# Daniel-Liu-c0deb0t/block-aligner

Hardware: AMD Instinct MI355X
Metric: GCUPS (DP cells/s) on 10 kbp DNA X-drop batch; bit-exact score+CIGAR vs AVX2 (higher is better)
Workload: dtype i16 (saturating lane scores) + i32 block offsets

## Files before the change

block_aligner_amd/csrc/ba_host.cpp:

```cpp
#include <hip/hip_runtime.h>

#include <algorithm>
#include <functional>
#include <cmath>
#include <cstdarg>
#include <cstdio>
#include <cstdlib>
#include <cstring>
#include <map>
#include <memory>
#include <string>
#include <vector>
#include <atomic>
#include <chrono>
#include <thread>

#include "../../include/block_aligner_hip.h"
#include "aa_matrices.inc"
#include "ba_extend.h"
#include "ba_stats.h"
#include "ba_params.h"

using ba::BatchParams;
using ba::BlockRec;
// ... 1500 lines not shown
        } else (void)hipGetLastError();
        out = (uint32_t*)at.devicePointer;
    }
    if (!out) {
        if (!b->compact.p) {
            b->compact_cap = std::max<uint64_t>(b->cap_cig / 3, 1u << 20);
            if (b->compact.alloc(b->compact_cap * 4)) return 1;
        }
        out = b->compact.as<uint32_t>(); cap = b->compact_cap;
    }
    HIP_TRY(ba_launch_cigar_offsets_and_compact(b->stream, b->cig_ops.as<uint32_t>(), b->cig_off.as<uint64_t>(), b->cig_len.as<uint32_t>(),
                                                b->h_order.empty() ? nullptr : b->dev_of.as<uint32_t>(), b->compact_off.as<uint64_t>(), out,
                                                b->h_total, cap, b->n));
    b->compacted = true; b->compact_host = pinned_out; b->compact_used_cap = cap;
    return 0;
}
int ba_batch_cigars(BaBatch* b, uint32_t* runs, uint64_t capacity) {
    if (!b) return fail("null batch");
    if (!(b->mode & BA_TRACE)) return fail("batch was created without BA_TRACE");
    if (!b->ran) return fail("ba_batch_run has not been called");
    HIP_TRY(hipSetDevice(b->device));
    if (b->compacted && b->retried == 0) {
        const unsigned long long total = *(volatile unsigned long long*)b->h_total;
        if (total <= b->compact_used_cap) {
            if (total > capacity) return fail("cigar buffer too small: need %llu entries", total);
            if (b->compact_host) { if (runs != b->compact_host && total) memcpy(runs, b->compact_host, total * 4); }
            else if (total) HIP_TRY(hipMemcpy(runs, b->compact.p, total * 4, hipMemcpyDeviceToHost));
            return 0;
        }
    }
    std::vector<uint32_t> len(b->n);
    if (d2h(b->cig_len, len.data(), b->n)) return 1;
    std::vector<uint64_t> out_off(b->n);
    uint64_t total = 0;
    if (b->h_order.empty()) for (uint32_t p = 0; p < b->n; p++) { out_off[p] = total; total += len[p]; }
    else {
        std::vector<uint32_t> dev_of(b->n);
        for (uint32_t s = 0; s < b->n; s++) dev_of[b->h_order[s]] = s;
        for (uint32_t p = 0; p < b->n; p++) { out_off[dev_of[p]] = total; total += len[dev_of[p]]; }
    }
    if (total > capacity) return fail("cigar buffer too small: need %llu entries", (unsigned long long)total);
    if (total == 0) return 0;
    DevBuf d_off, d_out;
    if (d_off.alloc(b->n * 8) || d_out.alloc(total * 4)) return 1;
    HIP_TRY(hipMemcpy(d_off.p, out_off.data(), b->n * 8, hipMemcpyHostToDevice));
    HIP_TRY(ba_launch_compact_cigars(b->stream, b->cig_ops.as<uint32_t>(), b->cig_off.as<uint64_t>(), b->cig_len.as<uint32_t>(),
                                     d_off.as<uint64_t>(), d_out.as<uint32_t>(), b->n));
    HIP_TRY(hipStreamSynchronize(b->stream));
    HIP_TRY(hipMemcpy(runs, d_out.p, total * 4, hipMemcpyDeviceToHost));
    return 0;
}
#ifdef BA_DEV
int ba_dev_lane_scan(int form, const int16_t* x, uint32_t n_cells, int gap_extend, int16_t* out) {
    if (form < 0 || form > 4 || !x || !out) return fail("ba_dev_lane_scan: bad arguments");
    const uint32_t per_wave = form <= 1 ? 512u : (form == 2 ? 128u : (form == 3 ? 64u : 32u));
    if (n_cells == 0 || n_cells % per_wave) return fail("ba_dev_lane_scan: %u cells are not whole waves of %u", n_cells, per_wave);
    if (gap_extend > 0 || gap_extend < -128) return fail("ba_dev_lane_scan: gap_extend %d", gap_extend);
    DevBuf dx, dout;
    if (dx.alloc((size_t)n_cells * 2) || dout.alloc((size_t)n_cells * 2)) return 1;
    HIP_TRY(hipMemcpy(dx.p, x, (size_t)n_cells * 2, hipMemcpyHostToDevice));
    HIP_TRY(ba_launch_lane_kat(nullptr, form, dx.as<short>(), dout.as<short>(), gap_extend, n_cells / per_wave));
    HIP_TRY(hipDeviceSynchronize());
    HIP_TRY(hipMemcpy(out, dout.p, (size_t)n_cells * 2, hipMemcpyDeviceToHost));
    return 0;
}
#endif
int ba_batch_prof(BaBatch* b, uint64_t out[128]) {
    if (!b) return fail("null batch");
    HIP_TRY(hipMemcpy(out, b->prof.p, 1024, hipMemcpyDeviceToHost));
    return 0;
}
int ba_batch_info(BaBatch* b, uint64_t out[4]) {
    if (!b) return fail("null batch");
    out[0] = (uint64_t)b->grid * b->wpw; out[1] = b->lds / b->wpw; out[2] = b->trace.bytes; out[3] = b->pool_bytes;
    return 0;
}
int ba_batch_spec_cells(BaBatch* b, uint64_t* cells) {
    if (!b || !cells) return fail("null argument");
    if (!b->ran) return fail("ba_batch_run has not been called");
    HIP_TRY(hipSetDevice(b->device));
    HIP_TRY(hipMemcpy(cells, (const char*)b->prof.p + 60 * 8, 8, hipMemcpyDeviceToHost));
    return 0;
}
int ba_batch_kernel(BaBatch* b) { return !b ? -1 : (b->small ? 3 : (b->quad ? 2 : (b->multi ? 1 : 0))); }
int ba_batch_geometry(BaBatch* b) { return !b ? -1 : (int)b->geom; }
int ba_batch_retried(BaBatch* b) { return b ? (int)b->retried : -1; }
int ba_batch_stats(BaBatch* b, BaAlignStats* out) {
    if (!b) return fail("null batch");
    if (!out) return fail("null argument");
    if (batch_stats_device(b, true)) return 1;
    HIP_TRY(hipMemcpy(out, b->stats.p, (size_t)b->n * sizeof(ba::AlignStats), hipMemcpyDeviceToHost));
    return 0;
}
int ba_batch_stats_ms(BaBatch* b, float* ms) {
    if (!b || !ms) return fail("null argument");
    *ms = b->stats_ms;
    return 0;
}
void ba_batch_destroy(BaBatch* b) { delete b; }

BaExtendBatch* ba_extend_batch_create(int kind, const void* matrix, Gaps gaps, SizeRange size, int32_t x_drop, uint32_t mode, const uint8_t* pool,
                                      const uint64_t* q_off, const uint32_t* q_len, const uint64_t* r_off, const uint32_t* r_len,
                                      const uint32_t* q_seed, const uint32_t* r_seed, const uint32_t* seed_len, const uint8_t* strand, uintptr_t n_seeds) {
    ExtSet S;
    if (!matrix) { fail("null argument"); return nullptr; }
    if (ext_check_params(kind, gaps, size, x_drop, mode) || ext_plan(kind, pool, q_off, q_len, r_off, r_len, q_seed, r_seed, seed_len, strand, n_seeds, S)) return nullptr;
    if (ensure_device()) return nullptr;
    std::unique_ptr<BaExtendBatch> e(new BaExtendBatch);
// ... 833 lines not shown
```

block_aligner_amd/csrc/ba_kernels.hip:

```cpp
#include "ba_driver.hpp"

#ifndef BA_KIND
#error "define BA_KIND"
#endif
#ifndef BA_PMAX
#error "define BA_PMAX"
#endif

#ifndef BA_SPECIAL
#define BA_SPECIAL 0
#endif

#define BA_CAT_(a, b, c, d) a##b##c##d
#define BA_CAT(a, b, c, d) BA_CAT_(a, b, c, d)
#if BA_BIG && BA_SPECIAL
#define BA_LAUNCH BA_CAT(ba_launch_bigs_k, BA_KIND, _p, BA_PMAX)
#define BA_OCC BA_CAT(ba_occupancy_bigs_k, BA_KIND, _p, BA_PMAX)
#elif BA_BIG
#define BA_LAUNCH BA_CAT(ba_launch_big_k, BA_KIND, _p, BA_PMAX)
#define BA_OCC BA_CAT(ba_occupancy_big_k, BA_KIND, _p, BA_PMAX)
#elif BA_SPECIAL
#define BA_LAUNCH BA_CAT(ba_launch_s_k, BA_KIND, _p, BA_PMAX)
#define BA_OCC BA_CAT(ba_occupancy_s_k, BA_KIND, _p, BA_PMAX)
#else
// ... 258 lines not shown
}
#endif

#if BA_PMAX == 1 && !BA_SPECIAL && !BA_BIG
#include "ba_quad.hpp"
template <bool TRACE, bool XDROP>
static hipError_t quad_grid(unsigned* grid) {
    const unsigned lds = ba::lds_table_bytes_h(BA_KIND) + ba::WAVES_PER_WG * 4 * ba::QUAD_SLOT_BYTES;
    int per_cu = 0, dev = 0;
    hipError_t e = hipOccupancyMaxActiveBlocksPerMultiprocessor(&per_cu, ba::k_quad<BA_KIND, TRACE, XDROP>, ba::WAVES_PER_WG * 64, lds);
    if (e != hipSuccess) return e;
    hipDeviceProp_t prop;
    if ((e = hipGetDevice(&dev)) != hipSuccess || (e = hipGetDeviceProperties(&prop, dev)) != hipSuccess) return e;
    if (per_cu < 1) per_cu = 1;
    if (per_cu * ba::WAVES_PER_WG > 32) per_cu = 32 / ba::WAVES_PER_WG;
    *grid = (unsigned)(prop.multiProcessorCount * per_cu);
    return hipSuccess;
}
template <bool TRACE, bool XDROP>
static hipError_t launch_quad(unsigned grid, hipStream_t s, const ba::BatchParams& bp) {
    const unsigned lds = ba::lds_table_bytes_h(BA_KIND) + ba::WAVES_PER_WG * 4 * ba::QUAD_SLOT_BYTES;
    ba::k_quad<BA_KIND, TRACE, XDROP><<<dim3(grid), dim3(ba::WAVES_PER_WG * 64), lds, s>>>(bp);
    return hipGetLastError();
}
extern "C" hipError_t BA_CAT(ba_launch_quad_k, BA_KIND, , )(int trace, int xdrop, unsigned grid, hipStream_t s, const ba::BatchParams* bp) {
    if (trace) return xdrop ? launch_quad<true, true>(grid, s, *bp) : launch_quad<true, false>(grid, s, *bp);
    return xdrop ? launch_quad<false, true>(grid, s, *bp) : launch_quad<false, false>(grid, s, *bp);
}
extern "C" hipError_t BA_CAT(ba_quad_grid_k, BA_KIND, , )(int trace, int xdrop, unsigned* grid) {
    if (trace) return xdrop ? quad_grid<true, true>(grid) : quad_grid<true, false>(grid);
    return xdrop ? quad_grid<false, true>(grid) : quad_grid<false, false>(grid);
}
#endif

#if BA_KIND == 0 && BA_PMAX == 1 && !BA_SPECIAL && !BA_BIG
__global__ void __launch_bounds__(64) k_traceback(const ba::BatchParams bp) {
    using namespace ba;
    __shared__ uint32_t words[4096];
    uint32_t st = 0, n = 0;
    if (bp.flags & (F_LOCAL | F_FQS)) {
        if (lane_id() == 0)
            n = traceback(bp.blocks + (uint64_t)bp.tb_slot * bp.blocks_stride, bp.tb_nblocks, bp.trace_arena + (uint64_t)bp.tb_slot * bp.trace_stride, bp.tb_i,
                          bp.tb_j, bp.pool + bp.q_off[0], bp.pool + bp.r_off[0], bp.flags, bp.cig_ops, bp.cig_off[0], bp.cig_off[1], &st);
    } else
        n = walk_wave<false>(bp.blocks + (uint64_t)bp.tb_slot * bp.blocks_stride, bp.tb_nblocks, bp.trace_arena + (uint64_t)bp.tb_slot * bp.trace_stride, bp.tb_i,
                             bp.tb_j, bp.pool + bp.q_off[0], bp.pool + bp.r_off[0], (bp.flags & F_CIGAR_EQ) != 0, bp.cig_ops, bp.cig_off[0], bp.cig_off[1], &st,
                             words, 4096u);
    if (lane_id() == 0) { bp.cig_len[0] = n; bp.status[0] = st; }
}

__global__ void __launch_bounds__(64) k_lane_kat(int form, const short* __restrict__ x, short* __restrict__ out, int gap_extend) {
    using namespace ba;
    const int lane = lane_id();
    if (form <= 1) {
        const short* xi = x + (size_t)blockIdx.x * 512 + lane * 8;
        int xr[4], r[4];
#pragma unroll
        for (int k = 0; k < 4; k++) xr[k] = pk((int)xi[2 * k], (int)xi[2 * k + 1]);
        const int ge2 = splat(gap_extend);
#pragma unroll
        for (int k = 0; k < 4; k++) r[k] = scan8_inreg(xr[k], ge2);
        int G[4], cs;
        if (form == 0) {
            const MultiConsts mc = make_multi_consts(lane & 15, gap_extend);
#pragma unroll
            for (int k = 0; k < 4; k++) G[k] = mc.G[k];
            scan8_chain(r, G[0]);
            cs = multi_carry(r[3], mc);
        } else {
            const SmallConsts mc = make_small_consts(lane & 3, gap_extend);
#pragma unroll
            for (int k = 0; k < 4; k++) G[k] = mc.G[k];
            scan8_chain(r, G[0]);
            cs = small_carry(r[3], mc, lane & 3);
        }
        short* oi = out + (size_t)blockIdx.x * 512 + lane * 8;
#pragma unroll
        for (int k = 0; k < 4; k++) { const int v = scan8_apply(r[k], cs, G[k], k == 3); oi[2 * k] = as_s(v).x; oi[2 * k + 1] = as_s(v).y; }
    } else {
        const int nl = form == 2 ? 64 : (form == 3 ? 32 : 16);
        const size_t base = (size_t)blockIdx.x * (size_t)(2 * nl);
        const int xv = lane < nl ? pk((int)x[base + 2 * lane], (int)x[base + 2 * lane + 1]) : 0;
        const FillConsts fc = make_fill_consts(lane, 0, gap_extend);
        const int v = form == 2 ? fast_scan<64>(xv, fc) : (form == 3 ? fast_scan<32>(xv, fc) : fast_scan<16>(xv, fc));
        if (lane < nl) { out[base + 2 * lane] = as_s(v).x; out[base + 2 * lane + 1] = as_s(v).y; }
    }
}
extern "C" hipError_t ba_launch_lane_kat(hipStream_t s, int form, const short* x, short* out, int gap_extend, unsigned waves) {
    k_lane_kat<<<dim3(waves), dim3(64), 0, s>>>(form, x, out, gap_extend);
    return hipGetLastError();
}

constexpr int WALK_WAVES = 4;
__global__ void __launch_bounds__(WALK_WAVES * 64) k_walk(const ba::BatchParams bp) {
    extern __shared__ __attribute__((aligned(16))) unsigned char walk_lds[];
    ba::traceback_all(bp, (uint32_t)ba::F_CIGAR_EQ, walk_lds + ((uint32_t)threadIdx.x >> 6) * ba::TB_LDS_BYTES);
}

__global__ void __launch_bounds__(WALK_WAVES * 64) k_walk_l2(const ba::BatchParams bp) {
    extern __shared__ __attribute__((aligned(16))) unsigned char walk_lds[];
    ba::traceback_all<true>(bp, (uint32_t)ba::F_CIGAR_EQ, walk_lds + ((uint32_t)threadIdx.x >> 6) * ba::TB_LDS_BYTES_L2);
}

__global__ void __launch_bounds__(WALK_WAVES * 64) k_walk_loc(const ba::BatchParams bp) {
    extern __shared__ __attribute__((aligned(16))) unsigned char walk_lds[];
    ba::traceback_all<true, true>(bp, (uint32_t)ba::F_CIGAR_EQ, walk_lds + ((uint32_t)threadIdx.x >> 6) * ba::TB_LDS_BYTES_LOC);
}
// ... 126 lines not shown
```

block_aligner_amd/csrc/ba_multi.hpp:

```cpp
#pragma once
#include "ba_quad.hpp"

namespace ba {
#ifndef MQ_SOLO_PRIO
#define MQ_SOLO_PRIO 2
#endif

template <int N>
__device__ __forceinline__ int row_bcast(int v) { return __builtin_amdgcn_update_dpp(v, v, 0x150 + N, 0xf, 0xf, false); }
__device__ __forceinline__ int row_shl1_keep(int last, int src) { return __builtin_amdgcn_update_dpp(last, src, 0x101, 0xf, 0xf, false); }
__device__ __forceinline__ int splat_hi(int x) { const s16x2 t = as_s(x); return as_i(s16x2{t.y, t.y}); }
__device__ __forceinline__ int splat_lo(int x) { const s16x2 t = as_s(x); return as_i(s16x2{t.x, t.x}); }

__device__ __forceinline__ int sel_mask(unsigned long long m, int a, int b) {
    int r;
    asm("v_cndmask_b32_e64 %0, %1, %2, %3" : "=v"(r) : "v"(b), "v"(a), "s"(m));
    return r;
}

template <int SL> __device__ __forceinline__ int slot_first(int v) {
    if constexpr (SL == 16) return row_bcast<0>(v);
    else if constexpr (SL == 64) return __builtin_amdgcn_readfirstlane(v);
    else return __builtin_amdgcn_ds_bpermute((lane_id() & 32) << 2, v);
}
template <int SL> __device__ __forceinline__ int slot_last(int v) {
    if constexpr (SL == 16) return row_bcast<15>(v);
    else if constexpr (SL == 64) return __builtin_amdgcn_readlane(v, 63);
    else return __builtin_amdgcn_ds_bpermute(((lane_id() & 32) + 31) << 2, v);
}
template <int SL> __device__ __forceinline__ int slot_shr1_z(int v, int l) {
    if constexpr (SL == 16) return row_shr1_z(v);
    else if constexpr (SL == 64) return wave_shr1_z(v);
    else { const int t = wave_shr1_z(v); return l == 0 ? 0 : t; }
}
template <int SL> __device__ __forceinline__ int slot_shl1_keep(int last, int src, int l) {
    if constexpr (SL == 16) return row_shl1_keep(last, src);
    else { const int t = __builtin_amdgcn_update_dpp(last, src, 0x130, 0xf, 0xf, false); return l == SL - 1 ? last : t; }
}

struct MultiConsts {
    int G[4];
    int laneKG, lanem1KG;
    int w0;
};

__device__ __forceinline__ MultiConsts make_multi_consts(int l, int gx) {
    MultiConsts mc;
    mc.laneKG = l * 8 * gx; mc.lanem1KG = l ? (l - 1) * 8 * gx : -32768;
#pragma unroll
    for (int k = 0; k < 4; k++) mc.G[k] = pk(max(-32768, (2 * k + 1) * gx), max(-32768, (2 * k + 2) * gx));
    mc.w0 = pk(0, l == 0 ? 0 : ((l & 1) ? max(-32768, 8 * l * gx) : 4 * gx));
    return mc;
}
template <int SL = 16>
__device__ __forceinline__ int multi_carry(int r3, const MultiConsts& mc, int l = 0) {
    if constexpr (SL == 16) {
        const int pm = wave_prefix_max16((int)as_s(r3).y - mc.laneKG);
        return vmax(scan8_splat_lo(add_row_shr1(pm, mc.lanem1KG)), mc.w0);
    } else {
        const int pm = SL == 64 ? wave_prefix_max((int)as_s(r3).y - mc.laneKG) : wave_prefix_max32((int)as_s(r3).y - mc.laneKG);
        const int cin = add_shr1(pm, mc.lanem1KG);
        return vmax(scan8_splat_lo(l == 0 ? -32768 : cin), mc.w0);
    }
}

struct MultiOut { int mx, act_max8, pas_max8, corner_new; };

template <int KIND, bool TRACE, int SPM = 0, int SL = 16>
__device__ __forceinline__ void multi_rect(const char* table, const FillConsts& fc, const MultiConsts& mc, int l, int (&Ad)[4], int (&Ac)[4],
                                           int (&Pd)[4], int (&Pr)[4], uint2 vb, uint32_t cb_lo, uint32_t cb_hi, int corner, int off_add,
                                           uint32_t* __restrict__ tout, bool store, MultiOut& o, int rz2 = 0, bool fqs_row0 = false, int* zout = nullptr) {
    uint32_t zacc[2] = {0, 0};
    const int offa = splat(off_add);
    int d[4], c[4], pd[4], pr[4];
#pragma unroll
    for (int k = 0; k < 4; k++) {
        d[k] = adds(Ad[k], offa); c[k] = adds(Ac[k], offa); pd[k] = adds(Pd[k], offa); pr[k] = adds(Pr[k], offa);
    }
    o.corner_new = slot_first<SL>(pd[3]) >> 16;
    ScoreKey<KIND> key[4];
#pragma unroll
    for (int k = 0; k < 4; k++) {
        const uint32_t w = k < 2 ? vb.x : vb.y;
        key[k] = make_key<KIND>((int)((w >> (16 * (k & 1))) & 0xffu), (int)((w >> (16 * (k & 1) + 8)) & 0xffu));
    }
    uint32_t kb[4] = {0, 0, 0, 0}, cbs_lo = 0, cbs_hi = 0;
    if constexpr (KIND == KIND_NUC) {
        const uint32_t tb = (uint32_t)(uintptr_t)table, k01 = nuc_keys2(vb.x), k23 = nuc_keys2(vb.y);
        kb[0] = add_word(k01, tb, 0); kb[1] = add_word(k01, tb, 1); kb[2] = add_word(k23, tb, 0); kb[3] = add_word(k23, tb, 1);
        cbs_lo = nuc_col_offsets(cb_lo); cbs_hi = nuc_col_offsets(cb_hi);
    }
    int dmax[4] = {0, 0, 0, 0}, tacc[8] = {0, 0, 0, 0, 0, 0, 0, 0};
    int nvD[4] = {0, 0, 0, 0}, nvR[4] = {0, 0, 0, 0};
    int holdD = 0, holdR = 0;
#pragma unroll
    for (int j = 0; j < STEP; j++) {
        const int cb = (int)(((j < 4 ? cb_lo : cb_hi) >> (8 * (j & 3))) & 0xffu);
        int sc[4];
#pragma unroll
        for (int k = 0; k < 4; k++) {
            if constexpr (KIND == KIND_NUC) sc[k] = lds_read_i32(add_byte(j < 4 ? cbs_lo : cbs_hi, kb[k], j));
            else sc[k] = fetch_score<KIND>(table, key[k], cb);
        }
        int prev = slot_shr1_z<SL>(d[3], l);
        if (j == 0) prev = l == 0 ? (int)((uint32_t)corner << 16) : prev;
        int d00[4];
        d00[0] = __builtin_amdgcn_alignbit(d[0], prev, 16);
#pragma unroll
        for (int k = 1; k < 4; k++) d00[k] = __builtin_amdgcn_alignbit(d[k], d[k - 1], 16);
        int d11[4], copen[4], cn[4], x[4], r[4];
#pragma unroll
        for (int k = 0; k < 4; k++) {
            d11[k] = adds(d00[k], sc[k]);
            if (SPM == 2 && k == 0) d11[0] = fqs_row0 ? (int)(((uint32_t)d11[0] & 0xffff0000u) | ((uint32_t)rz2 & 0xffffu)) : d11[0];
            if (SPM == 1) d11[k] = vmax(d11[k], rz2);
            copen[k] = adds(d[k], fc.go2);
            cn[k] = vmax(adds(c[k], fc.ge2), copen[k]);
            d11[k] = vmax(d11[k], cn[k]);
            x[k] = adds(d11[k], fc.ome2);
            r[k] = scan8_inreg(x[k], fc.ge2);
        }
        scan8_chain(r, mc.G[0]);
        const int cs = multi_carry<SL>(r[3], mc, l);
        int dn[4];
        uint32_t sC[4], sR[4], sCo[4], sRo[4];
#pragma unroll
        for (int k = 0; k < 4; k++) {
            r[k] = scan8_apply(r[k], cs, mc.G[k], k == 3);
            dn[k] = vmax(d11[k], r[k]);
            if (TRACE) {
                sC[k] = (uint32_t)subs(cn[k], dn[k]); sR[k] = (uint32_t)subs(r[k], dn[k]); sCo[k] = (uint32_t)subs(copen[k], cn[k]); sRo[k] = (uint32_t)subs(x[k], r[k]);
            }
            dmax[k] = vmax(dmax[k], dn[k]);
            d[k] = dn[k]; c[k] = cn[k];
        }
        if (TRACE && SPM == 1) {
#pragma unroll
            for (int p2 = 0; p2 < 2; p2++) {
                const uint32_t pZ = (uint32_t)__builtin_amdgcn_perm(subs(rz2, dn[2 * p2 + 1]), subs(rz2, dn[2 * p2]), 0x0b0a0908);
                zacc[p2] |= pZ & (0x01010101u << j);
            }
        }
        if (TRACE) {
#pragma unroll
            for (int p2 = 0; p2 < 2; p2++) {
                const uint32_t pC = (uint32_t)__builtin_amdgcn_perm((int)sC[2 * p2 + 1], (int)sC[2 * p2], 0x0b0a0908), pR = (uint32_t)__builtin_amdgcn_perm((int)sR[2 * p2 + 1], (int)sR[2 * p2], 0x0b0a0908);
                const uint32_t pCo = (uint32_t)__builtin_amdgcn_perm((int)sCo[2 * p2 + 1], (int)sCo[2 * p2], 0x0b0a0908), pRo = (uint32_t)__builtin_amdgcn_perm((int)sRo[2 * p2 + 1], (int)sRo[2 * p2], 0x0b0a0908);
                const uint32_t lo2 = bfi(0x55555555u, pC, pR), hi2 = bfi(0x55555555u, pCo, pRo);
                const uint32_t nib = bfi(0x33333333u, lo2, hi2);
                if (j & 1) tacc[2 * (j >> 1) + p2] = (int)bfi(0xF0F0F0F0u, nib, (uint32_t)tacc[2 * (j >> 1) + p2]);
                else tacc[2 * (j >> 1) + p2] = (int)nib;
            }
        }
        if (j & 1) { nvD[j >> 1] = __builtin_amdgcn_perm(dn[3], holdD, 0x07060302); nvR[j >> 1] = __builtin_amdgcn_perm(r[3], holdR, 0x07060302); }
        else { holdD = dn[3]; holdR = r[3]; }
    }
    if (TRACE) {
#ifndef MQ_X_NOTRSTORE
        if (store) { *(int4*)tout = int4{tacc[0], tacc[1], tacc[2], tacc[3]}; *(int4*)(tout + 4) = int4{tacc[4], tacc[5], tacc[6], tacc[7]}; }
#else
        asm volatile("" :: "v"(tacc[0]), "v"(tacc[1]), "v"(tacc[2]), "v"(tacc[3]), "v"(tacc[4]), "v"(tacc[5]), "v"(tacc[6]), "v"(tacc[7]));
#endif
    }
#pragma unroll
    for (int k = 0; k < 4; k++) {
        Pd[k] = slot_shl1_keep<SL>(nvD[k], pd[k], l); Pr[k] = slot_shl1_keep<SL>(nvR[k], pr[k], l);
        Ad[k] = d[k]; Ac[k] = c[k];
    }
    {
        const int ma = vmax(vmax(d[0], d[1]), vmax(d[2], d[3])), mb = vmax(vmax(Pd[0], Pd[1]), vmax(Pd[2], Pd[3]));
        const s16x2 sa = as_s(ma), sb = as_s(mb);
        const int xa = vmax(ma, as_i(s16x2{sa.y, sa.x})), xb = vmax(mb, as_i(s16x2{sb.y, sb.x}));
        const s16x2 rr = as_s(slot_first<SL>(__builtin_amdgcn_perm(xb, xa, 0x05040100)));
        o.act_max8 = rr.x; o.pas_max8 = rr.y;
    }
    const int mm = vmax(vmax(dmax[0], dmax[1]), vmax(dmax[2], dmax[3]));
    const int m32 = max(mm & 0xffff, (int)((uint32_t)mm >> 16));
    o.mx = slot_last<SL>(SL == 16 ? wave_prefix_max16(m32) : (SL == 64 ? wave_prefix_max(m32) : wave_prefix_max32(m32)));
    if constexpr (TRACE && SPM == 1) { zout[0] = (int)~zacc[0]; zout[1] = (int)~zacc[1]; }
}

enum { MR_PAIR = 0, MR_BEST_I, MR_BEST_J, MR_CELLS_LO, MR_CELLS_HI, MR_BUDGET, MR_STATUS, MR_TSLOT, MR_SI, MR_SJ, MR_DIR, MR_PREV_DIR, MR_OFF, MR_OFF_MAX,
       MR_BEST_MAX, MR_Y_DROP, MR_X_ITER, MR_D_CORNER, MR_NSTEPS, MR_TRACE_TOP, MR_NBLOCKS, MR_SEL, MR_WORDS };
__device__ __forceinline__ int mq_load(const char* p) { return __hip_atomic_load((const int*)p, BA_RLX_AGENT); }

#ifndef MQ_PARTIAL_MB
#define MQ_PARTIAL_MB 256
#endif
#ifndef MQ_WAVES_EU
#define MQ_WAVES_EU 4
#endif
template <int PMAX, int KIND, bool TRACE, bool XDROP, int SPM = 0, int MBP = 128, int WPW = WAVES_PER_WG, int EU = MQ_WAVES_EU>
__global__ void __launch_bounds__(WPW * 64, (PMAX >= 16 ? 2 : EU)) k_multi(const BatchParams bp) {
    constexpr uint32_t MB = (uint32_t)MBP;
    constexpr int SL = MBP / 8, NSLOT = 64 / SL;
    constexpr uint32_t ALLM = (1u << NSLOT) - 1u;
    constexpr uint32_t ARR = 2u * MB, BUFL = 4u * ARR, BUFA = BUFL + 64u, SLOTA = 2u * BUFA + 128u;
    static_assert((MBP == 128 || MBP == 256 || MBP == 512) && NSLOT * SLOTA <= MQ_WAVE_BYTES && NSLOT * 2u * BUFL <= MQ_LDS_SCALARS && (MBP == 128 || SPM == 0), "k_multi slot geometry");
    static_assert(MBP != 128 || (BUFA == MQ_BUF_BYTES && SLOTA == MQ_SLOT_BYTES), "ba_params.h");
    constexpr uint32_t MQ_TW = (STEP * MB / 8) * (SPM == 1 ? 2u : 1u);
    constexpr int TB_LB = SPM ? (int)TB_LANE_BYTES_LOC : (int)TB_LANE_BYTES_L2;
    constexpr uint32_t TB_MASK = SPM ? ~0u : (uint32_t)F_CIGAR_EQ;
    extern __shared__ __attribute__((aligned(16))) char smem[];
    const int lane = lane_id(), l = lane & (SL - 1), g = lane / SL;
    const int wave = uni((int)threadIdx.x >> 6);
    {
        char* tab = smem;
        if (KIND == KIND_NUC) {
            nuc_table_fill(tab, bp.matrix, (int)threadIdx.x, WPW * 64);
        } else {
            const int nbytes = KIND == KIND_AA ? 27 * 32 : 2;
            for (int k = (int)threadIdx.x; k < nbytes; k += WPW * 64) tab[k] = (char)bp.matrix[k];
        }
    }
    __syncthreads();
    constexpr uint32_t LCLS = (uint32_t)PMAX * 128u;
    constexpr uint32_t ab = lds_array_bytes_h(LCLS);
    char* base = smem + lds_table_bytes_h(KIND) + (uint32_t)wave * mq_wave_bytes_h(LCLS);
    WaveLds L;
    L.D_col = (short*)(base + 0 * ab); L.C_col = (short*)(base + 1 * ab);
    L.D_row = (short*)(base + 2 * ab); L.R_row = (short*)(base + 3 * ab);
    L.misc = (short*)(base + 4 * ab);
    L.table = smem;
    const int gx = bp.gap_extend;
    const uint32_t stride = bp.tb_stride;
    const bool batch_traceback = TRACE && stride > 0;
#if defined(BA_TIMING) || defined(BA_ENDHIST)
    if (bp.prof && blockIdx.x == 0 && wave == 1 && is_lane(0)) atomicMax(bp.prof + 43, (unsigned long long)__builtin_amdgcn_s_memrealtime());
#endif
#ifdef BA_TIMING
    unsigned long long t_solo = 0, t_quad = 0, t_wait = 0, n_solo = 0, n_quad = 0;
#endif
// ... 159 lines not shown
                        uint32_t f = 0, head = 0;
                        if ((uint32_t)lane < bp.slots_per_wave) f = __hip_atomic_load(bp.slot_free + s_slot + lane, BA_RLX_AGENT);
                        if (is_lane(0)) head = __hip_atomic_load(bp.tb_ctrl + 32, BA_RLX_AGENT);
                        const unsigned long long fm = __ballot(f != 0);
                        if (fm) {
                            s_slot += (uint32_t)__builtin_ctzll(fm);
                            if (is_lane(0)) __hip_atomic_store(bp.slot_free + s_slot, 0u, BA_RLX_AGENT);
                            break;
                        }
                        head = (uint32_t)uni((int)head);
                        if (head != seen) { seen = head; idle_n = 0; }
                        else if ((++idle_n & 2047u) == 0 && traceback_help_one<TB_LB>(bp, TB_MASK, (unsigned char*)base)) idle_n = 0;
                        __builtin_amdgcn_s_sleep(64);
                    }
#ifdef BA_TIMING
                    t_wait += __builtin_amdgcn_s_memtime() - tw_a;
#endif
                } else if (TRACE) {
                    s_slot += (uint32_t)solo;
                }
            } else {
                const int rv = lane < MR_WORDS ? mq_load(rec + 4 * lane) : 0;
#define BA_W(v, k) __builtin_amdgcn_readlane(v, k)
                const uint32_t s_sel = (uint32_t)BA_W(rv, MR_SEL);
                const char* live_b = smem_s + (s_sel ^ 1u) * BUFA; const char* ck_b = smem_s + s_sel * BUFA;
                const int cv = lane < 16 ? mq_load(ck_b + BUFL + 4 * lane) : 0;
                s_pair = (uint32_t)BA_W(rv, MR_PAIR); s_slot = (uint32_t)BA_W(rv, MR_TSLOT);
                st.si = (uint32_t)BA_W(rv, MR_SI); st.sj = (uint32_t)BA_W(rv, MR_SJ); st.dir = BA_W(rv, MR_DIR); st.prev_dir = BA_W(rv, MR_PREV_DIR);
                st.off = BA_W(rv, MR_OFF); st.off_max = BA_W(rv, MR_OFF_MAX); st.best_max = BA_W(rv, MR_BEST_MAX);
                st.y_drop_iter = (uint32_t)BA_W(rv, MR_Y_DROP); st.x_drop_iter = BA_W(rv, MR_X_ITER); st.D_corner = BA_W(rv, MR_D_CORNER);
                st.trace_top = (uint32_t)BA_W(rv, MR_TRACE_TOP); st.nblocks = (uint32_t)BA_W(rv, MR_NBLOCKS);
                const uint32_t ns = (uint32_t)BA_W(rv, MR_NSTEPS);
                st.best_i = (uint32_t)BA_W(rv, MR_BEST_I); st.best_j = (uint32_t)BA_W(rv, MR_BEST_J);
                st.cells = ((unsigned long long)(uint32_t)BA_W(rv, MR_CELLS_LO) | ((unsigned long long)(uint32_t)BA_W(rv, MR_CELLS_HI) << 32)) + (unsigned long long)ns * (STEP * MB);
                const uint32_t bud = (uint32_t)BA_W(rv, MR_BUDGET);
                st.step_budget = bud > ns ? bud - ns : 1u;
                st.status = (uint32_t)BA_W(rv, MR_STATUS);
                const int flag = BA_W(cv, 0);
                const bool ck_pre = flag != 0;
                st.ck_i = (uint32_t)BA_W(cv, 1); st.ck_j = (uint32_t)BA_W(cv, 2); st.ck_off = BA_W(cv, 3);
                st.ck_tt = (uint32_t)BA_W(cv, 4) + (flag ? MQ_TW : 0u); st.ck_nb = (uint32_t)BA_W(cv, 5) + (flag ? 1u : 0u);
                const int ck_dir = BA_W(cv, 6), ck_offadd = BA_W(cv, 7), ck_corner = BA_W(cv, 8);
#undef BA_W
                {
                    int reg[16], ckr[16];
                    const bool lr = st.dir == DIR_RIGHT, cr = ck_dir == DIR_RIGHT;
                    const uint32_t oAd = (lr ? 0u : 2 * ARR) + l * 16, oAc = (lr ? ARR : 3 * ARR) + l * 16, oPd = (lr ? 2 * ARR : 0u) + l * 16, oPr = (lr ? 3 * ARR : ARR) + l * 16;
                    const uint32_t cAd = (cr ? 0u : 2 * ARR) + l * 16, cAc = (cr ? ARR : 3 * ARR) + l * 16, cPd = (cr ? 2 * ARR : 0u) + l * 16, cPr = (cr ? 3 * ARR : ARR) + l * 16;
#pragma unroll
                    for (int k = 0; k < 4; k++) {
                        reg[k] = mq_load(live_b + oAd + 4 * k); reg[4 + k] = mq_load(live_b + oAc + 4 * k); reg[8 + k] = mq_load(live_b + oPd + 4 * k); reg[12 + k] = mq_load(live_b + oPr + 4 * k);
                        ckr[k] = mq_load(ck_b + cAd + 4 * k); ckr[4 + k] = mq_load(ck_b + cAc + 4 * k); ckr[8 + k] = mq_load(ck_b + cPd + 4 * k); ckr[12 + k] = mq_load(ck_b + cPr + 4 * k);
                    }
                    al.import_slot(reg, ckr, s_pair, ck_pre || MB < max_size, ck_pre, ck_dir, ck_offadd, ck_corner, st.ck_i, st.ck_j, st.best_i, st.best_j, st.ck_off);
                }
            }
            al.trace = bp.trace_arena + (uint64_t)s_slot * bp.trace_stride;
            al.blocks = bp.blocks + (uint64_t)s_slot * bp.blocks_stride;
            int keepv = 0;
            park<0>(keepv, (int)live_m); park<1>(keepv, (int)pend_m); park<2>(keepv, (int)w_next); park<3>(keepv, (int)w_end);
            park<4>(keepv, (more ? 1 : 0) | (fresh ? 2 : 0) | (to_end ? 4 : 0) | (drain ? 8 : 0)); park<5>(keepv, solo); park<6>(keepv, (int)s_pair); park<7>(keepv, (int)s_slot);
            BA_TSTAMP(tr_a);
            __builtin_amdgcn_s_setprio(MQ_SOLO_PRIO);
            st = al.run(s_pair, s_slot, batch_traceback, nullptr, fresh ? MM_FRESH : MM_RESUME, st, !to_end, !fresh && !to_end);
            __builtin_amdgcn_s_setprio(0);
            live_m = (uint32_t)unpark<0>(keepv); pend_m = (uint32_t)unpark<1>(keepv); w_next = (uint32_t)unpark<2>(keepv); w_end = (uint32_t)unpark<3>(keepv);
            { const int fl = unpark<4>(keepv); more = fl & 1; fresh = fl & 2; to_end = fl & 4; drain = fl & 8; }
            solo = unpark<5>(keepv); s_pair = (uint32_t)unpark<6>(keepv); s_slot = (uint32_t)unpark<7>(keepv);
            char* const smem_s2 = (char*)coldp_big() + (uint64_t)fill_wave_of() * MQ_WAVE_BYTES + (uint32_t)solo * SLOTA;
            char* const rec2 = smem_s2 + 2 * BUFA;
#ifdef BA_TIMING
            {
                const unsigned long long tr_b = __builtin_amdgcn_s_memtime();
                al.prof[45] += tr_b - tr_a; al.prof[46] += fresh ? 1 : 0;
                if (bp.prof && is_lane(0)) {
                    for (int k = 0; k < 48; k++) if (k != 17 && !(k >= 20 && k < 32) && !(k >= 40 && k < 44)) atomicAdd(bp.prof + k, al.prof[k]);
                    atomicAdd(bp.prof + (fresh ? 56 : (to_end ? 58 : 57)), tr_b - tr_a);
                }
            }
#endif
            pend_m &= ~(1u << solo);
            if (st.exited) {
                const bool rgt = st.dir == DIR_RIGHT;
                if (lane < SL) {
                    const int l8 = 8 * l;
                    const int4 a_d = *(const int4*)((rgt ? L.D_col : L.D_row) + l8), a_c = *(const int4*)((rgt ? L.C_col : L.R_row) + l8);
                    const int4 p_d = *(const int4*)((rgt ? L.D_row : L.D_col) + l8), p_r = *(const int4*)((rgt ? L.R_row : L.C_col) + l8);
                    char* b1 = smem_s2 + BUFA;
                    *(int4*)(b1 + l * 16) = a_d; *(int4*)(b1 + ARR + l * 16) = a_c; *(int4*)(b1 + 2 * ARR + l * 16) = p_d; *(int4*)(b1 + 3 * ARR + l * 16) = p_r;
                    if (MB < max_size) {
                        char* b0 = smem_s2;
                        *(int4*)(b0 + l * 16) = *(const int4*)(L.D_col + MB + l8); *(int4*)(b0 + ARR + l * 16) = *(const int4*)(L.C_col + MB + l8);
                        *(int4*)(b0 + 2 * ARR + l * 16) = *(const int4*)(L.D_row + MB + l8); *(int4*)(b0 + 3 * ARR + l * 16) = *(const int4*)(L.R_row + MB + l8);
                    }
                }
                if (is_lane(0)) {
                    char* b0 = smem_s2;
                    *(int4*)(b0 + BUFL) = int4{0, (int)st.ck_i, (int)st.ck_j, st.ck_off}; *(int4*)(b0 + BUFL + 16) = int4{(int)st.ck_tt, (int)st.ck_nb, DIR_RIGHT, 0};
                    *(int*)(b0 + BUFL + 32) = 0;
                    int* rc = (int*)rec2;
                    rc[MR_PAIR] = (int)s_pair; rc[MR_BEST_I] = (int)st.best_i; rc[MR_BEST_J] = (int)st.best_j; rc[MR_CELLS_LO] = (int)(uint32_t)st.cells; rc[MR_CELLS_HI] = (int)(uint32_t)(st.cells >> 32);
                    rc[MR_BUDGET] = (int)st.step_budget; rc[MR_STATUS] = (int)st.status; rc[MR_TSLOT] = (int)s_slot; rc[MR_SI] = (int)st.si; rc[MR_SJ] = (int)st.sj; rc[MR_DIR] = st.dir;
                    rc[MR_PREV_DIR] = st.prev_dir; rc[MR_OFF] = st.off; rc[MR_OFF_MAX] = st.off_max; rc[MR_BEST_MAX] = st.best_max; rc[MR_Y_DROP] = (int)st.y_drop_iter;
                    rc[MR_X_ITER] = st.x_drop_iter; rc[MR_D_CORNER] = st.D_corner; rc[MR_NSTEPS] = 0; rc[MR_TRACE_TOP] = (int)st.trace_top; rc[MR_NBLOCKS] = (int)st.nblocks; rc[MR_SEL] = 0;
                }
                lds_sync();
                live_m |= 1u << solo;
            } else live_m &= ~(1u << solo);
#ifdef BA_TIMING
            t_solo += __builtin_amdgcn_s_memtime() - ts_a; n_solo++;
#endif
        }
        if (!live_m) break;

        {
            BA_TSTAMP(tq_a);
            char* const slot_mem = wave_mem + (uint32_t)g * SLOTA;
            const int x_drop = bp.x_drop;
            FillConsts fq;
            fq.go2 = splat(bp.gap_open); fq.ge2 = splat(gx); fq.ome2 = splat(clamp16(bp.gap_open - gx));
            MultiConsts mc = make_multi_consts(l, gx);
            const uint64_t tcap64 = bp.trace_stride, bcap64 = bp.blocks_stride;
            const uint32_t tcap = (uint32_t)(tcap64 < 0x7fffffffull ? tcap64 : 0x7fffffffull), bcap = (uint32_t)(bcap64 < 0x7fffffffull ? bcap64 : 0x7fffffffull);
            const bool live = (live_m >> g) & 1u;
            const char* rec = slot_mem + 2 * BUFA;
#define BA_R(k) (live ? mq_load(rec + 4 * (k)) : 0)
            const uint32_t pair = (uint32_t)BA_R(MR_PAIR), tslot = (uint32_t)BA_R(MR_TSLOT);
            uint32_t si = (uint32_t)BA_R(MR_SI), sj = (uint32_t)BA_R(MR_SJ), y_drop = (uint32_t)BA_R(MR_Y_DROP);
            uint32_t trace_top = (uint32_t)BA_R(MR_TRACE_TOP), nblocks = (uint32_t)BA_R(MR_NBLOCKS), sel = (uint32_t)BA_R(MR_SEL);
            int dir = BA_R(MR_DIR), prev_dir = BA_R(MR_PREV_DIR), off = BA_R(MR_OFF), off_max = BA_R(MR_OFF_MAX), best_max = BA_R(MR_BEST_MAX);
            int x_iter = BA_R(MR_X_ITER), D_corner = BA_R(MR_D_CORNER);
#undef BA_R
            int A_d[4], A_c[4], P_d[4], P_r[4];
            {
                const char* b = slot_mem + (sel ^ 1u) * BUFA + l * 16;
#pragma unroll
                for (int k = 0; k < 4; k++) {
                    A_d[k] = live ? mq_load(b + 4 * k) : 0; A_c[k] = live ? mq_load(b + ARR + 4 * k) : 0;
                    P_d[k] = live ? mq_load(b + 2 * ARR + 4 * k) : 0; P_r[k] = live ? mq_load(b + 3 * ARR + 4 * k) : 0;
                }
            }
            char* const lbuf = base + (uint32_t)g * (2u * BUFL);
            int* const lsc = (int*)(base + MQ_LDS_SCALARS) + (uint32_t)g * MQ_LSC_INTS;
            lds_sync();
            const unsigned long long qa_r = TRACE ? 0ull : (unsigned long long)(bp.pool + (live ? bp.q_off[pair] : 0ull)), ra_r = TRACE ? 0ull : (unsigned long long)(bp.pool + (live ? bp.r_off[pair] : 0ull));
            const uint32_t qlen_r = (!TRACE && live) ? bp.q_len[pair] : 0u, rlen_r = (!TRACE && live) ? bp.r_len[pair] : 0u;
            if (TRACE && l == 0) {
                const unsigned long long qa = (unsigned long long)(bp.pool + (live ? bp.q_off[pair] : 0ull)), ra = (unsigned long long)(bp.pool + (live ? bp.r_off[pair] : 0ull));
                *(int4*)(lsc + 20) = int4{(int)(uint32_t)qa, (int)(uint32_t)(qa >> 32), (int)(uint32_t)ra, (int)(uint32_t)(ra >> 32)};
                *(int4*)(lsc + 24) = int4{live ? (int)bp.q_len[pair] : 0, live ? (int)bp.r_len[pair] : 0, (int)tslot, 0};
            }
            if (live) {
                const char* cb = slot_mem + sel * BUFA;
                char* d = lbuf + sel * BUFL + l * 16;
#pragma unroll
                for (int a = 0; a < 4; a++) {
                    const char* sp = cb + a * ARR + l * 16;
                    *(int4*)(d + a * ARR) = int4{mq_load(sp), mq_load(sp + 4), mq_load(sp + 8), mq_load(sp + 12)};
                }
                if (l < 9) lsc[sel * 9u + l] = mq_load(cb + BUFL + 4 * l);
            }
            lds_sync();
            uint2 pf_qv = {0, 0}, pf_rv = {0, 0}, pf_qc = {0, 0}, pf_rc = {0, 0}; bool pf_ok = false;
            bool leave = false;
            auto stage = [&](uint32_t which, uint32_t s_i, uint32_t s_j, int s_off, uint32_t s_tt, uint32_t s_nb, int s_dir, int s_offadd, int s_corner) {
                char* b = lbuf + which * BUFL + l * 16;
                *(int4*)(b) = int4{A_d[0], A_d[1], A_d[2], A_d[3]}; *(int4*)(b + ARR) = int4{A_c[0], A_c[1], A_c[2], A_c[3]};
                *(int4*)(b + 2 * ARR) = int4{P_d[0], P_d[1], P_d[2], P_d[3]}; *(int4*)(b + 3 * ARR) = int4{P_r[0], P_r[1], P_r[2], P_r[3]};
                if (l == 0) {
                    int* sc = lsc + which * 9u;
                    sc[0] = 1; sc[1] = (int)s_i; sc[2] = (int)s_j; sc[3] = s_off; sc[4] = (int)s_tt; sc[5] = (int)s_nb; sc[6] = s_dir; sc[7] = s_offadd; sc[8] = s_corner;
                }
            };
            do {
                const bool right = dir == DIR_RIGHT;
                int4 cA = {0, 0, 0, 0}, cB = {0, 0, 0, 0};
                if (TRACE) { cA = *(const int4*)(lsc + 20); cB = *(const int4*)(lsc + 24); }
                const uint8_t* const qp = TRACE ? (const uint8_t*)((unsigned long long)(uint32_t)cA.x | ((unsigned long long)(uint32_t)cA.y << 32)) : (const uint8_t*)qa_r;
                const uint8_t* const rp = TRACE ? (const uint8_t*)((unsigned long long)(uint32_t)cA.z | ((unsigned long long)(uint32_t)cA.w << 32)) : (const uint8_t*)ra_r;
                const uint32_t qlen = TRACE ? (uint32_t)cB.x : qlen_r, rlen = TRACE ? (uint32_t)cB.y : rlen_r;
                const uint32_t ri = right ? si : sj, rj = (right ? sj : si) + (MB - STEP);
                const uint32_t lenV = right ? qlen : rlen, lenC = right ? rlen : qlen;
                const bool q_out = si + MB > qlen, r_out = sj + MB > rlen;
                bool elig = XDROP || ri + MB <= lenV || rj + STEP <= lenC;
                if (TRACE) elig = elig && nblocks < bcap && trace_top + MQ_TW + 64 <= tcap;
                leave = live && !elig;
                const bool run = live && !leave;
                const int off_n = off_max;
                const int off_add = sat16(off - off_n);
                const int corner = (prev_dir != dir && prev_dir != DIR_GROW) ? sat16(D_corner + off_add) : 0;
#ifndef MQ_X_NOSTAGE
                if (live) stage(sel ^ 1u, si, sj, off_n, trace_top, nblocks, dir, off_add, corner);
#endif
                asm volatile("" : "+v"(mc.laneKG), "+v"(mc.lanem1KG), "+v"(mc.w0));
                uint32_t l8;
                asm volatile("v_mbcnt_lo_u32_b32 %0, -1, 0\n\tv_mbcnt_hi_u32_b32 %0, -1, %0" : "=v"(l8));
                l8 = (l8 & (uint32_t)(SL - 1)) * 8u;
                uint2 vb, cbv;
                {
                    const uint8_t* Vp = right ? qp : rp; const uint8_t* Cp = right ? rp : qp;
                    vb = right ? pf_qv : pf_rv; cbv = right ? pf_rc : pf_qc;
                    if (__any(run && !pf_ok)) {
                        if (run && !pf_ok) {
                            const uint32_t* vp = (const uint32_t*)(Vp + (ri + l8));
                            vb.x = vp[0]; vb.y = vp[1];
                            const uint32_t* cp = (const uint32_t*)(Cp + rj);
                            cbv.x = cp[0]; cbv.y = cp[1];
                        }
                    }
                    asm volatile("" : "+v"(vb.x), "+v"(vb.y));
                    if (run) {
                        const uint32_t* a = (const uint32_t*)(qp + (si + l8)); const uint32_t* b = (const uint32_t*)(rp + (sj + l8));
                        const uint32_t* cq = (const uint32_t*)(qp + si + MB); const uint32_t* cr = (const uint32_t*)(rp + sj + MB);
                        pf_qv.x = a[0]; pf_qv.y = a[1]; pf_rv.x = b[0]; pf_rv.y = b[1];
                        pf_qc.x = cq[0]; pf_qc.y = cq[1]; pf_rc.x = cr[0]; pf_rc.y = cr[1];
                        pf_ok = true;
                    }
                }
                uint32_t* tw = nullptr;
                if (TRACE) {
                    uint32_t ts = (uint32_t)cB.z; asm volatile("" : "+v"(ts));
                    tw = bp.trace_arena + (uint64_t)ts * bp.trace_stride + (trace_top + l8);
                    if (run && l == 0) {
                        BlockRec br;
                        br.i = (right ? ri : rj) | 0x80000000u;
                        br.j = right ? rj : ri; br.h = (uint16_t)(right ? MB : STEP); br.w = (uint16_t)(right ? STEP : MB);
                        br.trace_base = trace_top | (right ? 0x80000000u : 0u);
                        bp.blocks[(uint64_t)(uint32_t)cB.z * bp.blocks_stride + nblocks] = br;
                    }
                }
                MultiOut o;
                int zw[2] = {0, 0};
                multi_rect<KIND, TRACE, SPM, SL>(smem, fq, mc, l, A_d, A_c, P_d, P_r, vb, cbv.x, cbv.y, corner, off_add, tw, run, o, SPM ? splat(sat16(ZERO - off_n)) : 0,
                                             SPM == 2 && right && ri == 0u && l == 0, zw);
                if (TRACE && SPM == 1 && run) *(int2*)(tw - 8 * l + 128 + 2 * l) = int2{zw[0], zw[1]};

                const int right_max = right ? o.act_max8 : o.pas_max8, down_max = right ? o.pas_max8 : o.act_max8;
                const int new_off_max = off_n + o.mx - ZERO;
                const bool improve = new_off_max > best_max;
                const uint32_t new_y = improve ? 0u : y_drop + 1;
                bool stop = q_out && r_out;
                if (XDROP) stop = stop || (!improve && new_off_max < best_max - x_drop && x_iter >= 1);
                stop = stop || (!q_out && !r_out && 2 * MB <= max_size && new_y > MB / STEP - 1);
                const bool commit = run && !stop;
                leave = leave || (run && stop);
                {
                    const bool imp = commit && improve;
// ... 87 lines not shown
```

Baseline: 2267.

## Switch multi-lane DP registers to strided packed layout with new prefix scan

Changes the in-register packing of the 8 cells per lane from adjacent pairs to a strided layout (cells k and k+4 share a register). This lets the within-lane gap scan run as a short chain across registers, replacing the per-register scan8 plus chain and apply steps, and turns the diagonal shift into plain register moves. Permutes are added at import and export boundaries (LDS staging, checkpoint restore, trace nibble packing, key building) to convert between layouts. A new test form exercises the strided scan. The aim is fewer VALU ops per DP step, at the cost of extra perm instructions at block edges and a risk of layout mismatches breaking bit-exactness.

Measured after the change: 2299, median of 6. +1.4%, better.

```diff
diff --git a/block_aligner_amd/csrc/ba_host.cpp b/block_aligner_amd/csrc/ba_host.cpp
--- a/block_aligner_amd/csrc/ba_host.cpp
+++ b/block_aligner_amd/csrc/ba_host.cpp
@@ -1576,8 +1576,8 @@
 }
 #ifdef BA_DEV
 int ba_dev_lane_scan(int form, const int16_t* x, uint32_t n_cells, int gap_extend, int16_t* out) {
-    if (form < 0 || form > 4 || !x || !out) return fail("ba_dev_lane_scan: bad arguments");
-    const uint32_t per_wave = form <= 1 ? 512u : (form == 2 ? 128u : (form == 3 ? 64u : 32u));
+    if (form < 0 || form > 5 || !x || !out) return fail("ba_dev_lane_scan: bad arguments");
+    const uint32_t per_wave = (form <= 1 || form == 5) ? 512u : (form == 2 ? 128u : (form == 3 ? 64u : 32u));
     if (n_cells == 0 || n_cells % per_wave) return fail("ba_dev_lane_scan: %u cells are not whole waves of %u", n_cells, per_wave);
     if (gap_extend > 0 || gap_extend < -128) return fail("ba_dev_lane_scan: gap_extend %d", gap_extend);
     DevBuf dx, dout;
diff --git a/block_aligner_amd/csrc/ba_kernels.hip b/block_aligner_amd/csrc/ba_kernels.hip
--- a/block_aligner_amd/csrc/ba_kernels.hip
+++ b/block_aligner_amd/csrc/ba_kernels.hip
@@ -334,7 +334,16 @@
 __global__ void __launch_bounds__(64) k_lane_kat(int form, const short* __restrict__ x, short* __restrict__ out, int gap_extend) {
     using namespace ba;
     const int lane = lane_id();
-    if (form <= 1) {
+    if (form == 5) {
+        const short* xi = x + (size_t)blockIdx.x * 512 + lane * 8;
+        int xr[4], r[4];
+#pragma unroll
+        for (int k = 0; k < 4; k++) xr[k] = pk((int)xi[k], (int)xi[k + 4]);
+        multi_scan_strided(xr, r, make_multi_consts(lane & 15, gap_extend));
+        short* oi = out + (size_t)blockIdx.x * 512 + lane * 8;
+#pragma unroll
+        for (int k = 0; k < 4; k++) { oi[k] = as_s(r[k]).x; oi[k + 4] = as_s(r[k]).y; }
+    } else if (form <= 1) {
         const short* xi = x + (size_t)blockIdx.x * 512 + lane * 8;
         int xr[4], r[4];
 #pragma unroll
diff --git a/block_aligner_amd/csrc/ba_multi.hpp b/block_aligner_amd/csrc/ba_multi.hpp
--- a/block_aligner_amd/csrc/ba_multi.hpp
+++ b/block_aligner_amd/csrc/ba_multi.hpp
@@ -42,6 +42,8 @@
     int G[4];
     int laneKG, lanem1KG;
     int w0;
+    int K[4];
+    int f4, f4w;
 };
 
 __device__ __forceinline__ MultiConsts make_multi_consts(int l, int gx) {
@@ -49,19 +51,50 @@
     mc.laneKG = l * 8 * gx; mc.lanem1KG = l ? (l - 1) * 8 * gx : -32768;
 #pragma unroll
     for (int k = 0; k < 4; k++) mc.G[k] = pk(max(-32768, (2 * k + 1) * gx), max(-32768, (2 * k + 2) * gx));
-    mc.w0 = pk(0, l == 0 ? 0 : ((l & 1) ? max(-32768, 8 * l * gx) : 4 * gx));
+    const int W = l == 0 ? 0 : ((l & 1) ? max(-32768, 8 * l * gx) : 4 * gx);
+    mc.w0 = pk(0, W);
+#pragma unroll
+    for (int k = 0; k < 4; k++) mc.K[k] = splat(max(-32768, (k + 1) * gx));
+    mc.f4 = pk(0, max(-32768, 4 * gx)); mc.f4w = pk(0, max(-32768, W + 4 * gx));
     return mc;
 }
 template <int SL = 16>
-__device__ __forceinline__ int multi_carry(int r3, const MultiConsts& mc, int l = 0) {
+__device__ __forceinline__ int multi_carry_raw(int e, const MultiConsts& mc, int l = 0) {
     if constexpr (SL == 16) {
-        const int pm = wave_prefix_max16((int)as_s(r3).y - mc.laneKG);
-        return vmax(scan8_splat_lo(add_row_shr1(pm, mc.lanem1KG)), mc.w0);
+        const int pm = wave_prefix_max16((int)as_s(e).y - mc.laneKG);
+        return scan8_splat_lo(add_row_shr1(pm, mc.lanem1KG));
     } else {
-        const int pm = SL == 64 ? wave_prefix_max((int)as_s(r3).y - mc.laneKG) : wave_prefix_max32((int)as_s(r3).y - mc.laneKG);
+        const int pm = SL == 64 ? wave_prefix_max((int)as_s(e).y - mc.laneKG) : wave_prefix_max32((int)as_s(e).y - mc.laneKG);
         const int cin = add_shr1(pm, mc.lanem1KG);
-        return vmax(scan8_splat_lo(l == 0 ? -32768 : cin), mc.w0);
-    }
+        return scan8_splat_lo(l == 0 ? -32768 : cin);
+    }
+}
+template <int SL = 16>
+__device__ __forceinline__ int multi_carry(int r3, const MultiConsts& mc, int l = 0) { return vmax(multi_carry_raw<SL>(r3, mc, l), mc.w0); }
+template <int SL = 16>
+__device__ __forceinline__ void multi_scan_strided(const int (&x)[4], int (&r)[4], const MultiConsts& mc, int l = 0) {
+    r[0] = x[0];
+#pragma unroll
+    for (int k = 1; k < 4; k++) r[k] = vmax(x[k], adds(r[k - 1], mc.K[0]));
+    const int e = vmax(r[3], adds(scan8_splat_lo(r[3]), mc.K[3]));
+    const int a = adds(multi_carry_raw<SL>(e, mc, l), mc.f4);
+    const int cp = vmax(a, (int)((uint32_t)r[3] << 16));
+    const int c = vmax(cp, mc.K[3]), c3 = vmax(cp, mc.f4w);
+#pragma unroll
+    for (int k = 0; k < 4; k++) r[k] = vmax(r[k], adds(k == 3 ? c3 : c, mc.K[k]));
+}
+__device__ __forceinline__ void strided_to_pairs(int (&v)[4]) {
+    const int s0 = v[0], s1 = v[1], s2 = v[2], s3 = v[3];
+    v[0] = __builtin_amdgcn_perm(s1, s0, 0x05040100); v[1] = __builtin_amdgcn_perm(s3, s2, 0x05040100);
+    v[2] = __builtin_amdgcn_perm(s1, s0, 0x07060302); v[3] = __builtin_amdgcn_perm(s3, s2, 0x07060302);
+}
+__device__ __forceinline__ int4 pairs_to_strided(int4 c) {
+    return int4{__builtin_amdgcn_perm(c.z, c.x, 0x05040100), __builtin_amdgcn_perm(c.z, c.x, 0x07060302),
+                __builtin_amdgcn_perm(c.w, c.y, 0x05040100), __builtin_amdgcn_perm(c.w, c.y, 0x07060302)};
+}
+__device__ __forceinline__ void strided_bytes_to_cells(int& w0, int& w1) {
+    const int a = __builtin_amdgcn_perm(w1, w0, 0x06040200), b = __builtin_amdgcn_perm(w1, w0, 0x07050301);
+    w0 = a; w1 = b;
 }
 
 struct MultiOut { int mx, act_max8, pas_max8, corner_new; };
@@ -80,19 +113,16 @@
     o.corner_new = slot_first<SL>(pd[3]) >> 16;
     ScoreKey<KIND> key[4];
 #pragma unroll
-    for (int k = 0; k < 4; k++) {
-        const uint32_t w = k < 2 ? vb.x : vb.y;
-        key[k] = make_key<KIND>((int)((w >> (16 * (k & 1))) & 0xffu), (int)((w >> (16 * (k & 1) + 8)) & 0xffu));
-    }
+    for (int k = 0; k < 4; k++) key[k] = make_key<KIND>((int)((vb.x >> (8 * k)) & 0xffu), (int)((vb.y >> (8 * k)) & 0xffu));
     uint32_t kb[4] = {0, 0, 0, 0}, cbs_lo = 0, cbs_hi = 0;
     if constexpr (KIND == KIND_NUC) {
-        const uint32_t tb = (uint32_t)(uintptr_t)table, k01 = nuc_keys2(vb.x), k23 = nuc_keys2(vb.y);
+        const uint32_t tb = (uint32_t)(uintptr_t)table;
+        const uint32_t k01 = nuc_keys2((uint32_t)__builtin_amdgcn_perm((int)vb.y, (int)vb.x, 0x05010400)), k23 = nuc_keys2((uint32_t)__builtin_amdgcn_perm((int)vb.y, (int)vb.x, 0x07030602));
         kb[0] = add_word(k01, tb, 0); kb[1] = add_word(k01, tb, 1); kb[2] = add_word(k23, tb, 0); kb[3] = add_word(k23, tb, 1);
         cbs_lo = nuc_col_offsets(cb_lo); cbs_hi = nuc_col_offsets(cb_hi);
     }
     int dmax[4] = {0, 0, 0, 0}, tacc[8] = {0, 0, 0, 0, 0, 0, 0, 0};
     int nvD[4] = {0, 0, 0, 0}, nvR[4] = {0, 0, 0, 0};
-    int holdD = 0, holdR = 0;
 #pragma unroll
     for (int j = 0; j < STEP; j++) {
         const int cb = (int)(((j < 4 ? cb_lo : cb_hi) >> (8 * (j & 3))) & 0xffu);
@@ -105,9 +135,9 @@
         int prev = slot_shr1_z<SL>(d[3], l);
         if (j == 0) prev = l == 0 ? (int)((uint32_t)corner << 16) : prev;
         int d00[4];
-        d00[0] = __builtin_amdgcn_alignbit(d[0], prev, 16);
-#pragma unroll
-        for (int k = 1; k < 4; k++) d00[k] = __builtin_amdgcn_alignbit(d[k], d[k - 1], 16);
+        d00[0] = __builtin_amdgcn_alignbit(d[3], prev, 16);
+#pragma unroll
+        for (int k = 1; k < 4; k++) d00[k] = d[k - 1];
         int d11[4], copen[4], cn[4], x[4], r[4];
 #pragma unroll
         for (int k = 0; k < 4; k++) {
@@ -118,15 +148,12 @@
             cn[k] = vmax(adds(c[k], fc.ge2), copen[k]);
             d11[k] = vmax(d11[k], cn[k]);
             x[k] = adds(d11[k], fc.ome2);
-            r[k] = scan8_inreg(x[k], fc.ge2);
-        }
-        scan8_chain(r, mc.G[0]);
-        const int cs = multi_carry<SL>(r[3], mc, l);
+        }
+        multi_scan_strided<SL>(x, r, mc, l);
         int dn[4];
         uint32_t sC[4], sR[4], sCo[4], sRo[4];
 #pragma unroll
         for (int k = 0; k < 4; k++) {
-            r[k] = scan8_apply(r[k], cs, mc.G[k], k == 3);
             dn[k] = vmax(d11[k], r[k]);
             if (TRACE) {
                 sC[k] = (uint32_t)subs(cn[k], dn[k]); sR[k] = (uint32_t)subs(r[k], dn[k]); sCo[k] = (uint32_t)subs(copen[k], cn[k]); sRo[k] = (uint32_t)subs(x[k], r[k]);
@@ -151,9 +178,10 @@
                 if (j & 1) tacc[2 * (j >> 1) + p2] = (int)bfi(0xF0F0F0F0u, nib, (uint32_t)tacc[2 * (j >> 1) + p2]);
                 else tacc[2 * (j >> 1) + p2] = (int)nib;
             }
-        }
-        if (j & 1) { nvD[j >> 1] = __builtin_amdgcn_perm(dn[3], holdD, 0x07060302); nvR[j >> 1] = __builtin_amdgcn_perm(r[3], holdR, 0x07060302); }
-        else { holdD = dn[3]; holdR = r[3]; }
+            if (j & 1) strided_bytes_to_cells(tacc[2 * (j >> 1)], tacc[2 * (j >> 1) + 1]);
+        }
+        if (j < 4) { nvD[j] = dn[3]; nvR[j] = r[3]; }
+        else { nvD[j - 4] = __builtin_amdgcn_perm(dn[3], nvD[j - 4], 0x07060302); nvR[j - 4] = __builtin_amdgcn_perm(r[3], nvR[j - 4], 0x07060302); }
     }
     if (TRACE) {
 #ifndef MQ_X_NOTRSTORE
@@ -177,7 +205,11 @@
     const int mm = vmax(vmax(dmax[0], dmax[1]), vmax(dmax[2], dmax[3]));
     const int m32 = max(mm & 0xffff, (int)((uint32_t)mm >> 16));
     o.mx = slot_last<SL>(SL == 16 ? wave_prefix_max16(m32) : (SL == 64 ? wave_prefix_max(m32) : wave_prefix_max32(m32)));
-    if constexpr (TRACE && SPM == 1) { zout[0] = (int)~zacc[0]; zout[1] = (int)~zacc[1]; }
+    if constexpr (TRACE && SPM == 1) {
+        int z0 = (int)~zacc[0], z1 = (int)~zacc[1];
+        strided_bytes_to_cells(z0, z1);
+        zout[0] = z0; zout[1] = z1;
+    }
 }
 
 enum { MR_PAIR = 0, MR_BEST_I, MR_BEST_J, MR_CELLS_LO, MR_CELLS_HI, MR_BUDGET, MR_STATUS, MR_TSLOT, MR_SI, MR_SJ, MR_DIR, MR_PREV_DIR, MR_OFF, MR_OFF_MAX,
@@ -443,6 +475,10 @@
                         reg[k] = mq_load(live_b + oAd + 4 * k); reg[4 + k] = mq_load(live_b + oAc + 4 * k); reg[8 + k] = mq_load(live_b + oPd + 4 * k); reg[12 + k] = mq_load(live_b + oPr + 4 * k);
                         ckr[k] = mq_load(ck_b + cAd + 4 * k); ckr[4 + k] = mq_load(ck_b + cAc + 4 * k); ckr[8 + k] = mq_load(ck_b + cPd + 4 * k); ckr[12 + k] = mq_load(ck_b + cPr + 4 * k);
                     }
+#pragma unroll
+                    for (int a = 0; a < 4; a++) {
+                        strided_to_pairs(*(int(*)[4])(reg + 4 * a)); strided_to_pairs(*(int(*)[4])(ckr + 4 * a));
+                    }
                     al.import_slot(reg, ckr, s_pair, ck_pre || MB < max_size, ck_pre, ck_dir, ck_offadd, ck_corner, st.ck_i, st.ck_j, st.best_i, st.best_j, st.ck_off);
                 }
             }
@@ -475,14 +511,14 @@
                 const bool rgt = st.dir == DIR_RIGHT;
                 if (lane < SL) {
                     const int l8 = 8 * l;
-                    const int4 a_d = *(const int4*)((rgt ? L.D_col : L.D_row) + l8), a_c = *(const int4*)((rgt ? L.C_col : L.R_row) + l8);
-                    const int4 p_d = *(const int4*)((rgt ? L.D_row : L.D_col) + l8), p_r = *(const int4*)((rgt ? L.R_row : L.C_col) + l8);
+                    const int4 a_d = pairs_to_strided(*(const int4*)((rgt ? L.D_col : L.D_row) + l8)), a_c = pairs_to_strided(*(const int4*)((rgt ? L.C_col : L.R_row) + l8));
+                    const int4 p_d = pairs_to_strided(*(const int4*)((rgt ? L.D_row : L.D_col) + l8)), p_r = pairs_to_strided(*(const int4*)((rgt ? L.R_row : L.C_col) + l8));
                     char* b1 = smem_s2 + BUFA;
                     *(int4*)(b1 + l * 16) = a_d; *(int4*)(b1 + ARR + l * 16) = a_c; *(int4*)(b1 + 2 * ARR + l * 16) = p_d; *(int4*)(b1 + 3 * ARR + l * 16) = p_r;
                     if (MB < max_size) {
                         char* b0 = smem_s2;
-                        *(int4*)(b0 + l * 16) = *(const int4*)(L.D_col + MB + l8); *(int4*)(b0 + ARR + l * 16) = *(const int4*)(L.C_col + MB + l8);
-                        *(int4*)(b0 + 2 * ARR + l * 16) = *(const int4*)(L.D_row + MB + l8); *(int4*)(b0 + 3 * ARR + l * 16) = *(const int4*)(L.R_row + MB + l8);
+                        *(int4*)(b0 + l * 16) = pairs_to_strided(*(const int4*)(L.D_col + MB + l8)); *(int4*)(b0 + ARR + l * 16) = pairs_to_strided(*(const int4*)(L.C_col + MB + l8));
+                        *(int4*)(b0 + 2 * ARR + l * 16) = pairs_to_strided(*(const int4*)(L.D_row + MB + l8)); *(int4*)(b0 + 3 * ARR + l * 16) = pairs_to_strided(*(const int4*)(L.R_row + MB + l8));
                     }
                 }
                 if (is_lane(0)) {
@@ -583,7 +619,7 @@
 #ifndef MQ_X_NOSTAGE
                 if (live) stage(sel ^ 1u, si, sj, off_n, trace_top, nblocks, dir, off_add, corner);
 #endif
-                asm volatile("" : "+v"(mc.laneKG), "+v"(mc.lanem1KG), "+v"(mc.w0));
+                asm volatile("" : "+v"(mc.laneKG), "+v"(mc.lanem1KG), "+v"(mc.f4w));
                 uint32_t l8;
                 asm volatile("v_mbcnt_lo_u32_b32 %0, -1, 0\n\tv_mbcnt_hi_u32_b32 %0, -1, %0" : "=v"(l8));
                 l8 = (l8 & (uint32_t)(SL - 1)) * 8u;
```
